# srinix007/GaussianProcessRegression.jl

Measured on AMD Instinct MI355X. Metric: GP-fit+predict wall-time and K-build GB/s + POTRF TFLOP/s at N=32768, higher is better.
Workload: dtype f64; 1 GPU; C3 fit+posterior: SE+SE+WN, N=32768, d=8, np=8192; N=32768, d=8, np=8192, kernel=SE+SE+WN, nb=128, parallelism=replicas x1

## Files before the change

gaussianprocessregression.jl_amd/csrc/dag.hip:

```cpp
#include <algorithm>
#include <cstdint>

#include "common.hpp"

#ifdef DAG_TRACE
__device__ unsigned long long g_diag_ph[16];
#define DSTAMP_INIT() unsigned long long _dst_t = __builtin_amdgcn_s_memrealtime()
#define DSTAMP(i)                                                   \
  do {                                                              \
    __syncthreads();                                                \
    if (threadIdx.x == 0) {                                         \
      const unsigned long long _t = __builtin_amdgcn_s_memrealtime(); \
      atomicAdd(&g_diag_ph[i], _t - _dst_t);                        \
      if ((i) == 7) atomicAdd(&g_diag_ph[8], 1ull);                 \
      _dst_t = _t;                                                  \
    }                                                               \
  } while (0)
#define DSTAMPW(i)                                                  \
  do {                                                              \
    const unsigned long long _t = __builtin_amdgcn_s_memrealtime(); \
    if (threadIdx.x == 0) atomicAdd(&g_diag_ph[i], _t - _dst_t);    \
    _dst_t = _t;                                                    \
  } while (0)
extern "C" void gpr_debug_diag_phases(unsigned long long* out, int reset) {
  hipMemcpyFromSymbol(out, HIP_SYMBOL(g_diag_ph), sizeof(unsigned long long) * 16);
  if (reset) {
    unsigned long long z[16] = {};
    hipMemcpyToSymbol(HIP_SYMBOL(g_diag_ph), z, sizeof z);
  }
}
#endif

#include "diag_block.hpp"

#ifdef DAG_TRACE
__device__ int g_dag_trace[4096];
#define DTRACE(slot, v)                                                                   \
  do {                                                                                    \
    if (__builtin_amdgcn_readfirstlane(threadIdx.x >> 6) == 0)                            \
      __hip_atomic_store(&g_dag_trace[blockIdx.x * 8 + (slot)], (v), __ATOMIC_RELAXED,     \
                         __HIP_MEMORY_SCOPE_SYSTEM);                                      \
  } while (0)
extern "C" void gpr_debug_dag_trace(int* out, void* stream) {
  hipMemcpyFromSymbolAsync(out, HIP_SYMBOL(g_dag_trace), sizeof(int) * 4096, 0,
                           hipMemcpyDeviceToHost, (hipStream_t)stream);
  hipStreamSynchronize((hipStream_t)stream);
}
#define PROF(var, ...)                                  \
  do {                                                  \
    const unsigned long long _t0 = __builtin_amdgcn_s_memrealtime(); \
    __VA_ARGS__;                                        \
    var += __builtin_amdgcn_s_memrealtime() - _t0;      \
  } while (0)
#else
#define DTRACE(slot, v) \
  do {                  \
  } while (0)
#define PROF(var, ...) \
  do {                 \
    __VA_ARGS__;       \
  } while (0)
#endif

namespace {

constexpr int DT = 128;
constexpr int DTK = 16;
#ifndef DAG_DPB
#define DAG_DPB 5
#endif
static_assert(DAG_DPB == 4 || DAG_DPB == 5, "dag_accum is written for 4 or 5 LDS stages");
constexpr int DPB = DAG_DPB;
constexpr int DSTAGE = (DT + DT) * DTK;
constexpr int DLDS = DPB * DSTAGE;
constexpr int DINT = (DLDS + 2) * 8 <= 160 * 1024 ? DLDS : DLDS - 2;
constexpr int DALLOC = DINT + 2;
constexpr int DNCH = DTK / 2;
constexpr int DRPD = 64 / DNCH;
constexpr int DNDMA = DT / (4 * DRPD);
constexpr int DVM = 2 * DNDMA;
constexpr int DNP = DTK / 8;
static_assert(D2_LDS_QTAIL <= DLDS, "diagonal block must fit in the stage buffers");

typedef double d2 __attribute__((ext_vector_type(2)));

struct DagArgs {
  double* A;
  size_t lda;
  int n, nt;
  double* B;
  size_t ldb;
  int nrhs, ntr;
  double* winv;
  int kglob;
  int* info;
  int* sync;
  int* ustored;
  const unsigned* tasks;
  int ntasks;
  int lower;
  double* G;
  size_t ldg;
  int gbase;
  long long spin_limit;
  int mirror;
  const int* tbatch;
  size_t strA, strB, strW;
  int strS;
};

__device__ __forceinline__ int ld_sc1(const int* p) {
  return __hip_atomic_load(p, __ATOMIC_RELAXED, __HIP_MEMORY_SCOPE_AGENT);
}

template <int VM>
__device__ __forceinline__ void dag_vmcnt() {
  asm volatile("s_waitcnt vmcnt(%0)" ::"n"(VM) : "memory");
}

__device__ __forceinline__ int dag_swz(int row) { return (row >> 1) & 7; }
__device__ __forceinline__ int dag_idx(int row, int chunk) {
  return row * DTK + ((chunk ^ dag_swz(row)) << 1);
}

__device__ __forceinline__ int dag_mblk(int wm, int j) {
  return 4 * (j >> 1) + (wm ? 1 + (j & 1) : 3 * (j & 1));
}

template <bool TRI = false>
__device__ __forceinline__ void dag_accum(d4v (&acc)[4][4], const double* __restrict__ P,
                                          size_t ldp, int mv, const double* __restrict__ Q,
                                          size_t ldq, int nv, int nst, double* lds) {
  if (nst <= 0) return;
  const int tid = threadIdx.x, lane = tid & 63;
  const int w = __builtin_amdgcn_readfirstlane(tid >> 6);
  const int wm = w & 1, wn = w >> 1;
  const double* srcP[DNDMA];
  const double* srcQ[DNDMA];
#pragma unroll
  for (int r = 0; r < DNDMA; ++r) {
    const int row = DRPD * (4 * r + w) + lane / DNCH;
    const int c = (lane % DNCH) ^ dag_swz(row);
    srcP[r] = P + 2 * c + (size_t)min(row, mv - 1) * ldp;
    srcQ[r] = Q + 2 * c + (size_t)min(row, nv - 1) * ldq;
  }
  auto issue = [&](int s, int b) {
    double* base = lds + b * DSTAGE;
    const size_t ko = (size_t)min(s, nst - 1) * DTK;
#pragma unroll
    for (int r = 0; r < DNDMA; ++r) {
      __builtin_amdgcn_global_load_lds(srcP[r] + ko, base + (4 * r + w) * 128, 16, 0, 0);
      __builtin_amdgcn_global_load_lds(srcQ[r] + ko, base + DT * DTK + (4 * r + w) * 128, 16, 0, 0);
    }
  };
  auto read_frags = [&](d2 (&F)[DNP][8], int b) {
    const double* ps = lds + b * DSTAGE;
    const double* qs = ps + DT * DTK;
#pragma unroll
    for (int p = 0; p < DNP; ++p) {
      const int ch = (lane >> 4) + 4 * p;
#pragma unroll
      for (int i = 0; i < 4; ++i)
        F[p][i] = *reinterpret_cast<const d2*>(&qs[dag_idx(wn * 64 + i * 16 + (lane & 15), ch)]);
#pragma unroll
      for (int j = 0; j < 4; ++j) {
        const int mrow = TRI ? 16 * dag_mblk(wm, j) : wm * 64 + j * 16;
        F[p][4 + j] = *reinterpret_cast<const d2*>(&ps[dag_idx(mrow + (lane & 15), ch)]);
      }
    }
  };
  auto mfma_stage = [&](const d2 (&F)[DNP][8], int s) {
    (void)s;
#pragma unroll
    for (int j = 0; j < 4; ++j) {
      if (TRI && dag_mblk(wm, j) < s) continue;
#pragma unroll
      for (int p = 0; p < DNP; ++p)
#pragma unroll
        for (int h = 0; h < 2; ++h)
#pragma unroll
          for (int i = 0; i < 4; ++i)
            acc[i][j] = __builtin_amdgcn_mfma_f64_16x16x4f64(F[p][i][h], F[p][4 + j][h], acc[i][j], 0, 0, 0);
    }
  };
#if DAG_DPB == 5
  d2 F0[DNP][8], F1[DNP][8];
  auto ring = [](int b, int k) { return b + k >= DPB ? b + k - DPB : b + k; };
  auto period = [&](int s, int b) {
    __builtin_amdgcn_sched_barrier(0);
    __builtin_amdgcn_s_waitcnt(0xC07F);
    dag_vmcnt<DVM>();
    __builtin_amdgcn_s_barrier();
    issue(s + 4, ring(b, 4));
    read_frags(F1, ring(b, 1));
    mfma_stage(F0, s);
    if constexpr (!TRI) {
      __builtin_amdgcn_sched_group_barrier(0x008, 1, 0);
#pragma unroll
      for (int t = 0; t < DVM; ++t) {
        __builtin_amdgcn_sched_group_barrier(0x020, 1, 0);
        __builtin_amdgcn_sched_group_barrier(0x008, 2, 0);
      }
#pragma unroll
      for (int t = 0; t < 8 * DNP; ++t) {
        __builtin_amdgcn_sched_group_barrier(0x100, 1, 0);
        __builtin_amdgcn_sched_group_barrier(0x008, 2, 0);
      }
      __builtin_amdgcn_sched_group_barrier(0x008, 32 * DNP - 1 - 2 * DVM - 16 * DNP, 0);
    }
    issue(s + 5, b);
    read_frags(F0, ring(b, 2));
    mfma_stage(F1, s + 1);
    if constexpr (!TRI) {
#pragma unroll
      for (int t = 0; t < DVM; ++t) {
        __builtin_amdgcn_sched_group_barrier(0x020, 1, 0);
        __builtin_amdgcn_sched_group_barrier(0x008, 2, 0);
      }
#pragma unroll
      for (int t = 0; t < 8 * DNP; ++t) {
        __builtin_amdgcn_sched_group_barrier(0x100, 1, 0);
        __builtin_amdgcn_sched_group_barrier(0x008, 2, 0);
      }
      __builtin_amdgcn_sched_group_barrier(0x008, 32 * DNP - 2 * DVM - 16 * DNP, 0);
    }
  };
#pragma unroll
  for (int t = 0; t < DPB - 1; ++t) issue(t, t);
  dag_vmcnt<DVM * (DPB - 2)>();
  __builtin_amdgcn_s_barrier();
  read_frags(F0, 0);
  __builtin_amdgcn_s_waitcnt(0xC07F);
  int s = 0;
  for (int b = 0; s + 1 < nst; s += 2, b = ring(b, 2)) period(s, b);
#else
  auto step = [&](int s, d2 (&Fc)[DNP][8], d2 (&Fn)[DNP][8]) {
    __builtin_amdgcn_sched_barrier(0);
    __builtin_amdgcn_s_waitcnt(0xC07F);
    dag_vmcnt<DVM * (DPB - 3)>();
    __builtin_amdgcn_s_barrier();
    issue(s + DPB - 1, (s + DPB - 1) % DPB);
    read_frags(Fn, (s + 1) % DPB);
    mfma_stage(Fc, s);
    if constexpr (TRI) return;
#ifndef DAG_SCHED
#define DAG_SCHED 0
#endif
#if DAG_SCHED == 0
#pragma unroll
    for (int t = 0; t < DVM; ++t) {
      __builtin_amdgcn_sched_group_barrier(0x020, 1, 0);
      __builtin_amdgcn_sched_group_barrier(0x008, 1, 0);
    }
#pragma unroll
    for (int t = 0; t < 8 * DNP; ++t) {
      __builtin_amdgcn_sched_group_barrier(0x100, 1, 0);
      __builtin_amdgcn_sched_group_barrier(0x008, 2, 0);
    }
    __builtin_amdgcn_sched_group_barrier(0x008, 32 * DNP - DVM - 16 * DNP, 0);
#elif DAG_SCHED == 1
#pragma unroll
    for (int t = 0; t < DVM; ++t) {
      __builtin_amdgcn_sched_group_barrier(0x020, 1, 0);
      __builtin_amdgcn_sched_group_barrier(0x008, 2, 0);
    }
#pragma unroll
    for (int t = 0; t < 8 * DNP; ++t) {
      __builtin_amdgcn_sched_group_barrier(0x100, 1, 0);
      __builtin_amdgcn_sched_group_barrier(0x008, 2, 0);
    }
    __builtin_amdgcn_sched_group_barrier(0x008, 32 * DNP - 2 * DVM - 16 * DNP, 0);
#elif DAG_SCHED == 2
#pragma unroll
    for (int t = 0; t < 8 * DNP; ++t) {
      __builtin_amdgcn_sched_group_barrier(0x100, 1, 0);
      __builtin_amdgcn_sched_group_barrier(0x008, 1, 0);
    }
#pragma unroll
    for (int t = 0; t < DVM; ++t) {
      __builtin_amdgcn_sched_group_barrier(0x020, 1, 0);
      __builtin_amdgcn_sched_group_barrier(0x008, 2, 0);
    }
    __builtin_amdgcn_sched_group_barrier(0x008, 32 * DNP - 2 * DVM - 8 * DNP, 0);
#endif
  };
  d2 F0[DNP][8], F1[DNP][8];
#pragma unroll
  for (int t = 0; t < DPB - 1; ++t) issue(t, t);
  dag_vmcnt<DVM * (DPB - 2)>();
  __builtin_amdgcn_s_barrier();
  read_frags(F0, 0);
  __builtin_amdgcn_s_waitcnt(0xC07F);
  int s = 0;
  for (; s + 1 < nst; s += 2) {
    step(s, F0, F1);
    step(s + 1, F1, F0);
  }
#endif
  if (s < nst) mfma_stage(F0, s);
  dag_vmcnt<0>();
  __syncthreads();
}


__device__ __forceinline__ int dag_wait(const int* pa, const int* pb, int have, int cap,
                                        int* info, long long limit, int* sh) {
  if (__builtin_amdgcn_readfirstlane(threadIdx.x >> 6) == 0) {
    int v = 0;
    long long spins = 0;
    for (;;) {
      v = __builtin_amdgcn_readfirstlane(min(ld_sc1(pa), ld_sc1(pb)));
      if (v > have) break;
      if (++spins > limit) {
        atomicCAS(info, 0, -1);
        v = cap;
        break;
      }
      __builtin_amdgcn_s_sleep(2);
    }
    *sh = min(v, cap);
  }
  __builtin_amdgcn_fence(__ATOMIC_ACQUIRE, "workgroup");
  __syncthreads();
  const int r = __builtin_amdgcn_readfirstlane(*sh);
  __syncthreads();
  return r;
}

__device__ __forceinline__ void dag_publish(int* prog, int v) {
  asm volatile("s_waitcnt vmcnt(0)" ::: "memory");
  __syncthreads();
  if (__builtin_amdgcn_readfirstlane(threadIdx.x >> 6) == 0)
    __hip_atomic_store(prog, v, __ATOMIC_RELAXED, __HIP_MEMORY_SCOPE_AGENT);
}
// ... 47 lines not shown
#pragma unroll
  for (int ii = 0; ii < 4; ++ii)
#pragma unroll
    for (int r = 0; r < 4; ++r) {
      const int nn = wn * 64 + ii * 16 + (lane >> 4) + 4 * r;
#pragma unroll
      for (int jj = 0; jj < 4; ++jj) {
        const int mm = wm * 64 + jj * 16 + (lane & 15);
        if (mm < mv && nn < nv && (i != j || mm <= nn))
          T[(size_t)mm + (size_t)nn * a.ldg] = acc[ii][jj][r];
      }
    }
  double* Tm = a.G + (size_t)j * DT + (size_t)i * DT * a.ldg;
#pragma unroll
  for (int ii = 0; ii < 4; ++ii)
#pragma unroll
    for (int jj = 0; jj < 4; ++jj)
#pragma unroll
      for (int r = 0; r < 4; ++r) {
        const int nn = wn * 64 + ii * 16 + (lane >> 4) + 4 * r;
        const int mm = wm * 64 + jj * 16 + (lane & 15);
        if (mm < mv && nn < nv && (i != j || mm < nn))
          Tm[(size_t)nn + (size_t)mm * a.ldg] = acc[ii][jj][r];
      }
}

template <bool GRAM, bool BATCH>
__global__ __launch_bounds__(256, 1) void potrf_dag_kernel(DagArgs a0) {
  DagArgs a = a0;
  __shared__ double lds[DALLOC];
  int& s_task = reinterpret_cast<int*>(lds + DINT)[0];
  int& s_skip = reinterpret_cast<int*>(lds + DINT)[1];
  int& s_wait = reinterpret_cast<int*>(lds + DINT)[2];
  int s_fok = 0;
  const int tid = threadIdx.x, lane = tid & 63;
  const int w = __builtin_amdgcn_readfirstlane(tid >> 6);
  const int wm = w & 1, wn = w >> 1;
  int* colprog = a.sync + 2;
  int* rhsprog = colprog + a.nt;
  unsigned long long p_wait = 0, p_acc = 0, p_fac = 0, p_tri = 0, p_all = 0, p_n = 0;
#ifdef DAG_PROF_PUB
  unsigned long long p_pub = 0, p_tri_unused = 0;
#define p_tri p_tri_unused
#endif
  (void)p_wait; (void)p_acc; (void)p_fac; (void)p_tri; (void)p_all; (void)p_n;
#ifdef DAG_TRACE
  const unsigned long long p_start = __builtin_amdgcn_s_memrealtime();
#endif
  for (;;) {
    if (w == 0) {
      const int tk = atomicAdd(&a0.sync[0], lane == 0 ? 1 : 0);
      const int tk0 = __builtin_amdgcn_readlane(tk, 0);
      s_task = tk0;
      if (!BATCH) {
        s_skip = __builtin_amdgcn_readfirstlane(ld_sc1(a.info)) != 0;
      } else if (tk0 < a0.ntasks) {
        const int b = __builtin_amdgcn_readfirstlane(a0.tbatch[tk0]);
        s_skip = __builtin_amdgcn_readfirstlane(ld_sc1(a0.info + b)) != 0;
      }
    }
    __syncthreads();
    const int t = __builtin_amdgcn_readfirstlane(s_task);
    const bool skip = __builtin_amdgcn_readfirstlane(s_skip);
    DTRACE(0, t);
    DTRACE(1, 1);
    if (t >= a.ntasks) break;
    if (BATCH) {
      const int b = __builtin_amdgcn_readfirstlane(a0.tbatch[t]);
      a.A = a0.A + (size_t)b * a0.strA;
      a.B = a0.B + (size_t)b * a0.strB;
      a.winv = a0.winv + (size_t)b * a0.strW;
      a.info = a0.info + b;
      colprog = a0.sync + (size_t)b * a0.strS + 2;
      rhsprog = colprog + a.nt;
    }
    const unsigned code = __builtin_amdgcn_readfirstlane(a.tasks[t]);
    if (GRAM && t >= a.gbase) {
      if (!skip) dag_gram_task(a, (code >> 16) & 0x7fff, code & 0xffff, lds, &s_wait, p_wait, p_acc);
      ++p_n;
      __syncthreads();
      continue;
    }
    const bool rhs = code >> 31;
    const int i = (code >> 16) & 0x7fff, j = code & 0xffff;
    const bool diag = !rhs && i == j;
    double* T = rhs ? a.B + (size_t)i * DT + (size_t)j * DT * a.ldb
                    : a.A + (size_t)i * DT + (size_t)j * DT * a.lda;
    const size_t ldt = rhs ? a.ldb : a.lda;
    const double* Qcol = rhs ? a.B + (size_t)j * DT * a.ldb : a.A + (size_t)j * DT * a.lda;
    const double* Pcol = a.A + (size_t)i * DT * a.lda;
    int* pj = rhs ? rhsprog + j : colprog + j;
    const int mv = min(DT, a.n - i * DT);
    const int nv = min(DT, (rhs ? a.nrhs : a.n) - j * DT);
    if (!skip) {
      d4v acc[4][4];
#pragma unroll
      for (int ii = 0; ii < 4; ++ii)
#pragma unroll
        for (int r = 0; r < 4; ++r) {
          const int nn = wn * 64 + ii * 16 + (lane >> 4) + 4 * r;
          const double* col = T + (size_t)min(nn, nv - 1) * ldt;
#pragma unroll
          for (int jj = 0; jj < 4; ++jj) {
            const int mm = wm * 64 + jj * 16 + (lane & 15);
            const double c = col[min(mm, mv - 1)];
            acc[ii][jj][r] = (mm < mv && nn < nv) ? -c : 0.0;
          }
        }
      if (a.mirror && !rhs && !diag) {
        double* Tm = a.A + (size_t)j * DT + (size_t)i * DT * a.lda;
#pragma unroll
        for (int ii = 0; ii < 4; ++ii)
#pragma unroll
          for (int jj = 0; jj < 4; ++jj)
#pragma unroll
            for (int r = 0; r < 4; ++r) {
              const int nn = wn * 64 + ii * 16 + (lane >> 4) + 4 * r;
              const int mm = wm * 64 + jj * 16 + (lane & 15);
              if (mm < mv && nn < nv) Tm[(size_t)nn + (size_t)mm * a.lda] = -acc[ii][jj][r];
            }
      }
      DTRACE(1, 2);
      int done = (rhs && a.lower) ? j : 0;
      while (done < i) {
        int r = 0;
        PROF(p_wait, r = dag_wait(colprog + i, pj, done, i, a.info, a.spin_limit, &s_wait));
        PROF(p_acc, dag_accum(acc, Pcol + (size_t)done * DT, a.lda, mv, Qcol + (size_t)done * DT,
                              ldt, nv, (r - done) * (DT / DTK), lds));
        done = r;
      }
      if (diag) {
        double* S = lds;
#pragma unroll
        for (int ii = 0; ii < 4; ++ii)
#pragma unroll
          for (int r = 0; r < 4; ++r) {
            const int nn = wn * 64 + ii * 16 + (lane >> 4) + 4 * r;
#pragma unroll
            for (int jj = 0; jj < 4; ++jj) {
              const int mm = wm * 64 + jj * 16 + (lane & 15);
              if (mm <= nn) S[pk(mm, nn)] = nn < mv ? -acc[ii][jj][r] : (mm == nn ? 1.0 : 0.0);
            }
          }
        __syncthreads();
        DTRACE(1, 3);
        int f = 0;
        PROF(p_fac, f = dag_factor(S, mv, a.kglob + i * DT, a.winv + (size_t)i * DT * DT));
        if (f && w == 0) atomicCAS(a.info, 0, f);
        s_fok = f == 0;
        DTRACE(1, 4);
      } else {
        if (i > 0) {
#pragma unroll
          for (int ii = 0; ii < 4; ++ii)
#pragma unroll
            for (int r = 0; r < 4; ++r) {
              const int nn = wn * 64 + ii * 16 + (lane >> 4) + 4 * r;
#pragma unroll
              for (int jj = 0; jj < 4; ++jj) {
                const int mm = wm * 64 + jj * 16 + (lane & 15);
                if (mm < mv && nn < nv) T[(size_t)mm + (size_t)nn * ldt] = -acc[ii][jj][r];
              }
            }
        }
        asm volatile("s_waitcnt vmcnt(0)" ::: "memory");
        __builtin_amdgcn_fence(__ATOMIC_RELEASE, "workgroup");
        PROF(p_wait, dag_wait(colprog + i, colprog + i, i, i + 1, a.info, a.spin_limit, &s_wait));
#pragma unroll
        for (int ii = 0; ii < 4; ++ii)
#pragma unroll
          for (int jj = 0; jj < 4; ++jj) acc[ii][jj] = d4v{0.0, 0.0, 0.0, 0.0};
        const bool tri = mv == DT;
        if (tri)
          PROF(p_tri, dag_accum<true>(acc, a.winv + (size_t)i * DT * DT, DT, mv, T, ldt, nv, DT / DTK, lds));
        else
          PROF(p_tri, dag_accum(acc, a.winv + (size_t)i * DT * DT, DT, mv, T, ldt, nv, mv / DTK, lds));
#pragma unroll
        for (int ii = 0; ii < 4; ++ii)
#pragma unroll
          for (int r = 0; r < 4; ++r) {
            const int nn = wn * 64 + ii * 16 + (lane >> 4) + 4 * r;
#pragma unroll
            for (int jj = 0; jj < 4; ++jj) {
              const int mm = (tri ? 16 * dag_mblk(wm, jj) : wm * 64 + jj * 16) + (lane & 15);
              if (mm < mv && nn < nv) st_res<true>(&T[(size_t)mm + (size_t)nn * ldt], acc[ii][jj][r]);
            }
          }
      }
    } else if (a.mirror && !rhs && !diag) {
      double* Tm = a.A + (size_t)j * DT + (size_t)i * DT * a.lda;
      for (int e = tid; e < DT * DT; e += 256) {
        const int mm = e & (DT - 1), nn = e >> 7;
        if (mm < mv && nn < nv) Tm[(size_t)nn + (size_t)mm * a.lda] = T[(size_t)mm + (size_t)nn * ldt];
      }
    }
    DTRACE(1, 5);
#ifdef DAG_PROF_PUB
    if (diag) PROF(p_pub, dag_publish(pj, i + 1)); else dag_publish(pj, i + 1);
#else
    dag_publish(pj, i + 1);
#endif
    DTRACE(1, 6);
    if (diag && !skip && __builtin_amdgcn_readfirstlane(s_fok))
      dag_store_u(lds, T, a.lda, mv, a.ustored != nullptr);
    if (diag && a.ustored) dag_publish(a.ustored + i, 1);
    ++p_n;
  }
  DTRACE(1, 7);
#ifdef DAG_TRACE
  p_all = __builtin_amdgcn_s_memrealtime() - p_start;
  DTRACE(2, (int)p_wait);
  DTRACE(3, (int)p_acc);
  DTRACE(4, (int)p_fac);
#ifdef DAG_PROF_PUB
#undef p_tri
  DTRACE(5, (int)p_pub);
  (void)p_tri_unused;
#else
  DTRACE(5, (int)p_tri);
#endif
  DTRACE(6, (int)p_all);
  DTRACE(7, (int)p_n);
#endif
}

}

__global__ void dag_init_kernel(int* sync, int nt, int ntr, int solve, int lower) {
  for (int t = blockIdx.x * blockDim.x + threadIdx.x; t < nt + ntr; t += gridDim.x * blockDim.x)
    sync[2 + t] = t < nt ? (solve ? t + 1 : 0) : (lower ? t - nt : 0);
}

static long long dag_spin_limit(const gpr_ctx* ctx) {
#ifdef GPR_TESTING
  if (const char* sl = getenv("GPR_DAG_SPIN_LIMIT")) return std::max(1ll, atoll(sl));
#endif
  return ctx->dag_spin_limit;
}

bool dag_shape_ok(int n, int lda, const double* dA) {
  return n > 0 && n % 16 == 0 && lda % 16 == 0 && ((uintptr_t)dA & 127) == 0 && n <= DT * 32767;
}

bool dag_takes_whole(const gpr_ctx* ctx, int n, int lda, const double* dA) {
  (void)lda;
  (void)dA;
  return ctx->dag_mode && ctx->nb == DT && n > 0 &&
         n <= DT * 32767 - 16;
}

__global__ void dag_pad_in_kernel(const double* __restrict__ A, size_t lda, int n,
                                  double* __restrict__ W, int n2) {
  const size_t tot = (size_t)n2 * n2;
  for (size_t t = blockIdx.x * (size_t)blockDim.x + threadIdx.x; t < tot;
       t += (size_t)gridDim.x * blockDim.x) {
    const int r = (int)(t % n2), c = (int)(t / n2);
    if (r <= c) W[t] = c < n ? A[(size_t)r + (size_t)c * lda] : (r == c ? 1.0 : 0.0);
  }
}

__global__ void dag_pad_out_kernel(double* __restrict__ A, size_t lda, int n,
                                   const double* __restrict__ W, int n2) {
  const size_t tot = (size_t)n * n;
  for (size_t t = blockIdx.x * (size_t)blockDim.x + threadIdx.x; t < tot;
       t += (size_t)gridDim.x * blockDim.x) {
    const int r = (int)(t % n), c = (int)(t / n);
    if (r <= c) A[(size_t)r + (size_t)c * lda] = W[(size_t)r + (size_t)c * n2];
  }
}

int launch_potrf_dag_padded(gpr_ctx* ctx, double* dA, int n, int lda, double* dB, int nrhs,
                            int ldb) {
  const int n2 = (n + 15) / 16 * 16;
  hipStream_t st = ctx->stream;
// ... 3 lines not shown
    (void)hipGetLastError();
    return 1;
  }
  const int blocks = 2048;
  dag_pad_in_kernel<<<blocks, 256, 0, st>>>(dA, (size_t)lda, n, ctx->dpadA, n2);
  LAUNCH_CHECK(ctx);
  if (dB) {
    HIP_TRY(ctx, hipMemcpy2DAsync(ctx->dpadB, (size_t)n2 * sizeof(double), dB,
                                  (size_t)ldb * sizeof(double), (size_t)n * sizeof(double), nrhs,
                                  hipMemcpyDeviceToDevice, st));
    if (n2 > n)
      HIP_TRY(ctx, hipMemset2DAsync(ctx->dpadB + n, (size_t)n2 * sizeof(double), 0,
                                    (size_t)(n2 - n) * sizeof(double), nrhs, st));
  }
  const int rc = launch_potrf_dag(ctx, ctx->dpadA, n2, n2, dB ? ctx->dpadB : nullptr, nrhs, n2, 0,
                                  st, 0);
  if (rc) return rc < 0 ? rc : set_err(ctx, GPR_E_HIP, "padded tile-DAG: shape not eligible");
  dag_pad_out_kernel<<<blocks, 256, 0, st>>>(dA, (size_t)lda, n, ctx->dpadA, n2);
  LAUNCH_CHECK(ctx);
  if (dB)
    HIP_TRY(ctx, hipMemcpy2DAsync(dB, (size_t)ldb * sizeof(double), ctx->dpadB,
                                  (size_t)n2 * sizeof(double), (size_t)n * sizeof(double), nrhs,
                                  hipMemcpyDeviceToDevice, st));
  return 0;
}

int launch_potrf_dag(gpr_ctx* ctx, double* dA, int n, int lda, double* dB, int nrhs, int ldb,
                     int kglob, hipStream_t st, int flags, double* dG, int ldg) {
  const bool solve = flags & DAG_SOLVE, lower = flags & DAG_LOWER, gram = flags & DAG_GRAM;
  const bool mirror = flags & DAG_MIRROR;
  if ((solve || lower) && (!dB || kglob)) return 1;
  if (mirror && (solve || kglob)) return 1;
  if (gram && (!lower || !dG || ldg < n || nrhs != n)) return 1;
  if (ctx->nb != DT || n <= 0 || n % 16 || lda % 16 || ((uintptr_t)dA & 127) || n > DT * 32767 ||
      kglob % DT)
    return 1;
  if (dB && (nrhs <= 0 || ldb % 16 || ((uintptr_t)dB & 127) || nrhs > DT * 65535)) return 1;
  const int nt = (n + DT - 1) / DT, ntr = dB ? (nrhs + DT - 1) / DT : 0;
  GPR_TRY(ensure_winv(ctx, kglob + n, DT));
  if (ctx->dag_nt != nt || ctx->dag_ntr != ntr || ctx->dag_flags != (flags & ~DAG_MIRROR) ||
      ctx->dag_lag_built != ctx->dag_zlag) {
    std::vector<unsigned> tasks;
    tasks.reserve((size_t)nt * (nt + 1) + (size_t)nt * ntr);
    const int lag = solve || !lower ? 0 : std::min(ctx->dag_zlag, nt);
    auto rhs_row = [&](int i) {
      for (int c = 0; c < (lower ? std::min(ntr, i + 1) : ntr); ++c)
        tasks.push_back(0x80000000u | ((unsigned)i << 16) | (unsigned)c);
    };
    for (int i = 0; i < nt; ++i) {
      if (!solve)
        for (int j = i; j < nt; ++j) tasks.push_back(((unsigned)i << 16) | (unsigned)j);
      if (i - lag >= 0) rhs_row(i - lag);
    }
    for (int i = std::max(nt - lag, 0); i < nt; ++i) rhs_row(i);
    if (gram)
      for (int j = 0; j < nt; ++j)
        for (int i = 0; i <= j; ++i) tasks.push_back(((unsigned)i << 16) | (unsigned)j);
    if (ctx->dag_tasks) {
      HIP_TRY(ctx, hipStreamSynchronize(ctx->stream));
      HIP_TRY(ctx, hipFree(ctx->dag_tasks));
    }
    ctx->dag_tasks = nullptr;
    ctx->dag_nt = ctx->dag_ntr = -1;
    HIP_TRY(ctx, hipMalloc((void**)&ctx->dag_tasks, tasks.size() * sizeof(unsigned)));
    HIP_TRY(ctx, hipMemcpy(ctx->dag_tasks, tasks.data(), tasks.size() * sizeof(unsigned),
                           hipMemcpyHostToDevice));
    ctx->dag_ntasks = (int)tasks.size();
    ctx->dag_nt = nt;
    ctx->dag_ntr = ntr;
    ctx->dag_flags = flags & ~DAG_MIRROR;
// ... 58 lines not shown
      hook_ev = nullptr;
    }
    (void)hipGetLastError();
  }
  const double flops = (solve ? 0.0 : (double)n * n * n / 3.0) +
                       (lower ? (double)n * n * n / 3.0 : (double)n * n * (dB ? nrhs : 0)) +
                       (gram ? (double)n * n * n / 3.0 : 0.0);
  {
    hipStream_t ls = ctx->ls;
    ctx->ls = st;
    TimerScope ts(ctx, solve ? TC_DAG_SOLVE : TC_DAG, flops);
    if (gram)
      potrf_dag_kernel<true, false><<<grid, 256, 0, st>>>(a);
    else
      potrf_dag_kernel<false, false><<<grid, 256, 0, st>>>(a);
    ctx->ls = ls;
    const hipError_t le = hipGetLastError();
    if (le != hipSuccess) {
      if (hook_ev) hipEventDestroy(hook_ev);
      return set_err(ctx, GPR_E_HIP, "tile-DAG launch: %s", hipGetErrorString(le));
    }
  }
  if (hook) {
    hook(ctx->dag_hook_user, dA, n, lda, ctx->dag_sync + 2, a.ustored, nt, hook_ev);
    if (hook_ev) hipEventDestroy(hook_ev);
  }
  return 0;
}

int launch_potrf_dag_batch(gpr_ctx* ctx, double* dA, size_t strA, int n, int lda, double* dB,
                           size_t strB, int nrhs, int ldb, int nbatch, int* info_out) {
  hipStream_t st = ctx->stream;
  if (nbatch <= 0) return 0;
  if (n <= 0 || n % 16 || lda % 16 || strA % 16 || ((uintptr_t)dA & 127) || n > DT * 32767)
    return 1;
  if (dB && (nrhs <= 0 || ldb % 16 || strB % 16 || ((uintptr_t)dB & 127) || nrhs > DT * 65535))
    return 1;
  const int nt = (n + DT - 1) / DT, ntr = dB ? (nrhs + DT - 1) / DT : 0;
  std::vector<unsigned> tasks;
  std::vector<int> tb;
  const size_t per = (size_t)nt * (nt + 1) / 2 + (size_t)nt * ntr;
  tasks.reserve(per * nbatch);
  tb.reserve(per * nbatch);
  for (int i = 0; i < nt; ++i) {
    for (int b = 0; b < nbatch; ++b)
      for (int j = i; j < nt; ++j) {
        tasks.push_back(((unsigned)i << 16) | (unsigned)j);
        tb.push_back(b);
      }
    for (int b = 0; b < nbatch; ++b)
      for (int c = 0; c < ntr; ++c) {
        tasks.push_back(0x80000000u | ((unsigned)i << 16) | (unsigned)c);
        tb.push_back(b);
      }
  }
  const int ntasks = (int)tasks.size();
  const int strS = 2 + nt + ntr;
  const size_t nW = (size_t)nbatch * nt * DT * DT;
  const size_t nI = (size_t)ntasks * 2 + (size_t)nbatch * strS + (size_t)nbatch;
  GPR_TRY(ensure_buf(ctx, &ctx->dagb, &ctx->dagb_cap, nW + (nI + 1) / 2 + 1));
  double* W = ctx->dagb;
  unsigned* dtasks = reinterpret_cast<unsigned*>(W + nW);
  int* dtb = reinterpret_cast<int*>(dtasks + ntasks);
  int* dsync = dtb + ntasks;
  int* dinfo = dsync + (size_t)nbatch * strS;
  HIP_TRY(ctx, hipMemcpyAsync(dtasks, tasks.data(), sizeof(unsigned) * ntasks, hipMemcpyHostToDevice, st));
  HIP_TRY(ctx, hipMemcpyAsync(dtb, tb.data(), sizeof(int) * ntasks, hipMemcpyHostToDevice, st));
  HIP_TRY(ctx, hipMemsetAsync(dsync, 0, sizeof(int) * ((size_t)nbatch * strS + nbatch), st));
  if (ctx->ncu <= 0) {
// ... 44 lines not shown
```

Baseline: 3.349 GP jobs/s (fit N=32768 + posterior mean/var np=8192, per GPU).

## Stage triangular-solve Q operand directly into LDS instead of via global round-trip

For full-size diagonal-triangle tiles in the DAG Cholesky/TRSM kernel, the negated accumulator is written straight into the LDS Q stages of the ring buffer rather than stored to global memory and reloaded. The prologue then only DMAs the W-inverse (P) operand, and the first period waits on fewer outstanding loads. The task-code and batch-index loads are also hoisted into the ticket-fetch wave to save a reload. Extra trace instrumentation is added under DAG_TRACE. This relies on LDS stage layout matching the swizzle and on T no longer being written to global for that wave half, which is a correctness risk.

```diff
diff --git a/gaussianprocessregression.jl_amd/csrc/dag.hip b/gaussianprocessregression.jl_amd/csrc/dag.hip
--- a/gaussianprocessregression.jl_amd/csrc/dag.hip
+++ b/gaussianprocessregression.jl_amd/csrc/dag.hip
@@ -1,5 +1,6 @@
 #include <algorithm>
 #include <cstdint>
+#include <type_traits>
 
 #include "common.hpp"
 
@@ -52,13 +53,44 @@
     __VA_ARGS__;                                        \
     var += __builtin_amdgcn_s_memrealtime() - _t0;      \
   } while (0)
+__device__ int g_dag_trace2[4096];
+#define DTRACE2(slot, v)                                                                  \
+  do {                                                                                    \
+    if (__builtin_amdgcn_readfirstlane(threadIdx.x >> 6) == 0)                            \
+      __hip_atomic_store(&g_dag_trace2[blockIdx.x * 8 + (slot)], (v), __ATOMIC_RELAXED,    \
+                         __HIP_MEMORY_SCOPE_SYSTEM);                                      \
+  } while (0)
+extern "C" void gpr_debug_dag_trace2(int* out, void* stream) {
+  hipMemcpyFromSymbolAsync(out, HIP_SYMBOL(g_dag_trace2), sizeof(int) * 4096, 0,
+                           hipMemcpyDeviceToHost, (hipStream_t)stream);
+  hipStreamSynchronize((hipStream_t)stream);
+}
+#define PLAP0() (_lap = __builtin_amdgcn_s_memrealtime())
+#define PLAP(var)                                                   \
+  do {                                                              \
+    const unsigned long long _t = __builtin_amdgcn_s_memrealtime(); \
+    var += _t - _lap;                                               \
+    _lap = _t;                                                      \
+  } while (0)
+#define PDRAIN() asm volatile("s_waitcnt vmcnt(0)" ::: "memory")
+#define P_WPRO &p_wpro
 #else
+#define P_WPRO nullptr
 #define DTRACE(slot, v) \
   do {                  \
   } while (0)
 #define PROF(var, ...) \
   do {                 \
     __VA_ARGS__;       \
+  } while (0)
+#define PLAP0() \
+  do {          \
+  } while (0)
+#define PLAP(var) \
+  do {            \
+  } while (0)
+#define PDRAIN() \
+  do {           \
   } while (0)
 #endif
 
@@ -127,11 +159,16 @@
   return 4 * (j >> 1) + (wm ? 1 + (j & 1) : 3 * (j & 1));
 }
 
-template <bool TRI = false>
+template <bool TRI = false, bool QL = false>
 __device__ __forceinline__ void dag_accum(d4v (&acc)[4][4], const double* __restrict__ P,
                                           size_t ldp, int mv, const double* __restrict__ Q,
-                                          size_t ldq, int nv, int nst, double* lds) {
+                                          size_t ldq, int nv, int nst, double* lds,
+                                          unsigned long long* p_pro = nullptr) {
   if (nst <= 0) return;
+#ifdef DAG_TRACE
+  const unsigned long long t_in = __builtin_amdgcn_s_memrealtime();
+#endif
+  (void)p_pro;
   const int tid = threadIdx.x, lane = tid & 63;
   const int w = __builtin_amdgcn_readfirstlane(tid >> 6);
   const int wm = w & 1, wn = w >> 1;
@@ -153,6 +190,12 @@
       __builtin_amdgcn_global_load_lds(srcQ[r] + ko, base + DT * DTK + (4 * r + w) * 128, 16, 0, 0);
     }
   };
+  auto issue_p = [&](int s, int b) {
+    double* base = lds + b * DSTAGE;
+#pragma unroll
+    for (int r = 0; r < DNDMA; ++r)
+      __builtin_amdgcn_global_load_lds(srcP[r] + (size_t)s * DTK, base + (4 * r + w) * 128, 16, 0, 0);
+  };
   auto read_frags = [&](d2 (&F)[DNP][8], int b) {
     const double* ps = lds + b * DSTAGE;
     const double* qs = ps + DT * DTK;
@@ -186,10 +229,10 @@
 #if DAG_DPB == 5
   d2 F0[DNP][8], F1[DNP][8];
   auto ring = [](int b, int k) { return b + k >= DPB ? b + k - DPB : b + k; };
-  auto period = [&](int s, int b) {
+  auto period = [&](int s, int b, auto first) {
     __builtin_amdgcn_sched_barrier(0);
     __builtin_amdgcn_s_waitcnt(0xC07F);
-    dag_vmcnt<DVM>();
+    dag_vmcnt<(QL && decltype(first)::value) ? DNDMA : DVM>();
     __builtin_amdgcn_s_barrier();
     issue(s + 4, ring(b, 4));
     read_frags(F1, ring(b, 1));
@@ -225,14 +268,28 @@
       __builtin_amdgcn_sched_group_barrier(0x008, 32 * DNP - 2 * DVM - 16 * DNP, 0);
     }
   };
-#pragma unroll
-  for (int t = 0; t < DPB - 1; ++t) issue(t, t);
-  dag_vmcnt<DVM * (DPB - 2)>();
+  static_assert(!QL || TRI, "LDS-resident Q stages: the W-product only (nst = 8 > DPB - 1)");
+#pragma unroll
+  for (int t = 0; t < DPB - 1; ++t) {
+    if constexpr (QL)
+      issue_p(t, t);
+    else
+      issue(t, t);
+  }
+  dag_vmcnt<(QL ? DNDMA : DVM) * (DPB - 2)>();
   __builtin_amdgcn_s_barrier();
   read_frags(F0, 0);
   __builtin_amdgcn_s_waitcnt(0xC07F);
-  int s = 0;
-  for (int b = 0; s + 1 < nst; s += 2, b = ring(b, 2)) period(s, b);
+#ifdef DAG_TRACE
+  if (p_pro) *p_pro += __builtin_amdgcn_s_memrealtime() - t_in;
+#endif
+  int s = 0, b = 0;
+  if constexpr (QL) {
+    period(0, 0, std::true_type{});
+    s = 2;
+    b = 2;
+  }
+  for (; s + 1 < nst; s += 2, b = ring(b, 2)) period(s, b, std::false_type{});
 #else
   auto step = [&](int s, d2 (&Fc)[DNP][8], d2 (&Fn)[DNP][8]) {
     __builtin_amdgcn_sched_barrier(0);
@@ -284,6 +341,7 @@
     __builtin_amdgcn_sched_group_barrier(0x008, 32 * DNP - 2 * DVM - 8 * DNP, 0);
 #endif
   };
+  static_assert(!QL, "LDS-resident Q stages: the ring of five only");
   d2 F0[DNP][8], F1[DNP][8];
 #pragma unroll
   for (int t = 0; t < DPB - 1; ++t) issue(t, t);
@@ -300,6 +358,24 @@
   if (s < nst) mfma_stage(F0, s);
   dag_vmcnt<0>();
   __syncthreads();
+}
+
+#ifndef DAG_Q_LDS
+#define DAG_Q_LDS 1
+#endif
+constexpr bool DAG_QLDS = DAG_DPB == 5 && DAG_Q_LDS;
+__device__ __forceinline__ void dag_q_to_lds(const d4v (&acc)[4][4], double* lds, int wn, int lane) {
+  int l = lane;
+  asm volatile("" : "+v"(l));
+  const int kk = l & 15;
+#pragma unroll
+  for (int r = 0; r < 4; ++r) {
+    double* q = lds + DT * DTK + dag_idx(wn * 64 + (l >> 4) + 4 * r, kk >> 1) + (kk & 1);
+#pragma unroll
+    for (int ii = 0; ii < 4; ++ii)
+#pragma unroll
+      for (int jj = 0; jj < 4; ++jj) q[jj * DSTAGE + ii * 16 * DTK] = -acc[ii][jj][r];
+  }
 }
 
 
@@ -413,6 +489,7 @@
   int& s_task = reinterpret_cast<int*>(lds + DINT)[0];
   int& s_skip = reinterpret_cast<int*>(lds + DINT)[1];
   int& s_wait = reinterpret_cast<int*>(lds + DINT)[2];
+  int& s_code = reinterpret_cast<int*>(lds + DINT)[3];
   int s_fok = 0;
   const int tid = threadIdx.x, lane = tid & 63;
   const int w = __builtin_amdgcn_readfirstlane(tid >> 6);
@@ -427,27 +504,32 @@
   (void)p_wait; (void)p_acc; (void)p_fac; (void)p_tri; (void)p_all; (void)p_n;
 #ifdef DAG_TRACE
   const unsigned long long p_start = __builtin_amdgcn_s_memrealtime();
+  unsigned long long p_tkt = 0, p_ld = 0, p_mir = 0, p_bst = 0, p_wpro = 0, p_fin = 0, _lap = 0;
 #endif
   for (;;) {
+    PLAP0();
     if (w == 0) {
       const int tk = atomicAdd(&a0.sync[0], lane == 0 ? 1 : 0);
       const int tk0 = __builtin_amdgcn_readlane(tk, 0);
       s_task = tk0;
-      if (!BATCH) {
-        s_skip = __builtin_amdgcn_readfirstlane(ld_sc1(a.info)) != 0;
-      } else if (tk0 < a0.ntasks) {
-        const int b = __builtin_amdgcn_readfirstlane(a0.tbatch[tk0]);
-        s_skip = __builtin_amdgcn_readfirstlane(ld_sc1(a0.info + b)) != 0;
+      if (tk0 < a0.ntasks) {
+        const int b = BATCH ? __builtin_amdgcn_readfirstlane(a0.tbatch[tk0]) : 0;
+        const unsigned cd = a0.tasks[tk0];
+        const int sk = ld_sc1(a0.info + b);
+        s_code = __builtin_amdgcn_readfirstlane(cd);
+        s_skip = (__builtin_amdgcn_readfirstlane(sk) != 0) | (b << 1);
       }
     }
     __syncthreads();
     const int t = __builtin_amdgcn_readfirstlane(s_task);
-    const bool skip = __builtin_amdgcn_readfirstlane(s_skip);
+    const int skipb = __builtin_amdgcn_readfirstlane(s_skip);
+    const bool skip = skipb & 1;
+    const unsigned code = __builtin_amdgcn_readfirstlane(s_code);
     DTRACE(0, t);
     DTRACE(1, 1);
     if (t >= a.ntasks) break;
     if (BATCH) {
-      const int b = __builtin_amdgcn_readfirstlane(a0.tbatch[t]);
+      const int b = skipb >> 1;
       a.A = a0.A + (size_t)b * a0.strA;
       a.B = a0.B + (size_t)b * a0.strB;
       a.winv = a0.winv + (size_t)b * a0.strW;
@@ -455,7 +537,7 @@
       colprog = a0.sync + (size_t)b * a0.strS + 2;
       rhsprog = colprog + a.nt;
     }
-    const unsigned code = __builtin_amdgcn_readfirstlane(a.tasks[t]);
+    PLAP(p_tkt);
     if (GRAM && t >= a.gbase) {
       if (!skip) dag_gram_task(a, (code >> 16) & 0x7fff, code & 0xffff, lds, &s_wait, p_wait, p_acc);
       ++p_n;
@@ -488,6 +570,8 @@
             acc[ii][jj][r] = (mm < mv && nn < nv) ? -c : 0.0;
           }
         }
+      PDRAIN();
+      PLAP(p_ld);
       if (a.mirror && !rhs && !diag) {
         double* Tm = a.A + (size_t)j * DT + (size_t)i * DT * a.lda;
 #pragma unroll
@@ -500,6 +584,8 @@
               const int mm = wm * 64 + jj * 16 + (lane & 15);
               if (mm < mv && nn < nv) Tm[(size_t)nn + (size_t)mm * a.lda] = -acc[ii][jj][r];
             }
+        PDRAIN();
+        PLAP(p_mir);
       }
       DTRACE(1, 2);
       int done = (rhs && a.lower) ? j : 0;
@@ -530,8 +616,13 @@
         if (f && w == 0) atomicCAS(a.info, 0, f);
         s_fok = f == 0;
         DTRACE(1, 4);
+        PLAP0();
       } else {
-        if (i > 0) {
+        PLAP0();
+        const bool tri = mv == DT;
+        const bool qlds = DAG_QLDS && tri;
+        if (qlds && wm == 0) dag_q_to_lds(acc, lds, wn, lane);
+        if (i > 0 && !(qlds && wm == 0)) {
 #pragma unroll
           for (int ii = 0; ii < 4; ++ii)
 #pragma unroll
@@ -544,18 +635,21 @@
               }
             }
         }
-        asm volatile("s_waitcnt vmcnt(0)" ::: "memory");
+        if (!qlds) asm volatile("s_waitcnt vmcnt(0)" ::: "memory");
         __builtin_amdgcn_fence(__ATOMIC_RELEASE, "workgroup");
+        PLAP(p_bst);
         PROF(p_wait, dag_wait(colprog + i, colprog + i, i, i + 1, a.info, a.spin_limit, &s_wait));
 #pragma unroll
         for (int ii = 0; ii < 4; ++ii)
 #pragma unroll
           for (int jj = 0; jj < 4; ++jj) acc[ii][jj] = d4v{0.0, 0.0, 0.0, 0.0};
-        const bool tri = mv == DT;
         if (tri)
-          PROF(p_tri, dag_accum<true>(acc, a.winv + (size_t)i * DT * DT, DT, mv, T, ldt, nv, DT / DTK, lds));
+          PROF(p_tri, dag_accum<true, DAG_QLDS>(acc, a.winv + (size_t)i * DT * DT, DT, mv, T, ldt, nv,
+                                                DT / DTK, lds, P_WPRO));
         else
-          PROF(p_tri, dag_accum(acc, a.winv + (size_t)i * DT * DT, DT, mv, T, ldt, nv, mv / DTK, lds));
+          PROF(p_tri, dag_accum(acc, a.winv + (size_t)i * DT * DT, DT, mv, T, ldt, nv, mv / DTK, lds,
+                                P_WPRO));
+        PLAP0();
 #pragma unroll
         for (int ii = 0; ii < 4; ++ii)
 #pragma unroll
@@ -576,12 +670,16 @@
       }
     }
     DTRACE(1, 5);
+#ifdef DAG_TRACE
+    if (skip) PLAP0();
+#endif
 #ifdef DAG_PROF_PUB
     if (diag) PROF(p_pub, dag_publish(pj, i + 1)); else dag_publish(pj, i + 1);
 #else
     dag_publish(pj, i + 1);
 #endif
     DTRACE(1, 6);
+    PLAP(p_fin);
     if (diag && !skip && __builtin_amdgcn_readfirstlane(s_fok))
       dag_store_u(lds, T, a.lda, mv, a.ustored != nullptr);
     if (diag && a.ustored) dag_publish(a.ustored + i, 1);
@@ -602,6 +700,12 @@
 #endif
   DTRACE(6, (int)p_all);
   DTRACE(7, (int)p_n);
+  DTRACE2(0, (int)p_tkt);
+  DTRACE2(1, (int)p_ld);
+  DTRACE2(2, (int)p_mir);
+  DTRACE2(3, (int)p_bst);
+  DTRACE2(4, (int)p_wpro);
+  DTRACE2(5, (int)p_fin);
 #endif
 }
 
```

Measured after the change: 3.362 GP jobs/s (fit N=32768 + posterior mean/var np=8192, per GPU), median of 6. About the same (+0.4%).

## Hand-schedule DAG GEMM inner loop with inline-asm LDS DMA and precomputed addresses

Applied to the files above, without the earlier changes.

Rewrites the dag_accum inner pipeline. Global-to-LDS loads now go through inline asm with a scalar base and a 32-bit per-lane offset, and LDS fragment addresses are precomputed. The 5-stage ring is fully unrolled with compile-time buffer indices, and DMA pieces are interleaved explicitly between MFMAs. The aim is to cut per-iteration address arithmetic and VGPR pressure and to get a tighter MFMA/DMA interleave. In exchange it adds a leading-dimension limit so the 32-bit offsets stay valid (larger lda falls back off the DAG path), drops the 4-stage variant, and carries the risks of hand-written m0 asm.

```diff
diff --git a/gaussianprocessregression.jl_amd/csrc/dag.hip b/gaussianprocessregression.jl_amd/csrc/dag.hip
--- a/gaussianprocessregression.jl_amd/csrc/dag.hip
+++ b/gaussianprocessregression.jl_amd/csrc/dag.hip
@@ -1,5 +1,6 @@
 #include <algorithm>
 #include <cstdint>
+#include <type_traits>
 
 #include "common.hpp"
 
@@ -66,11 +67,8 @@
 
 constexpr int DT = 128;
 constexpr int DTK = 16;
-#ifndef DAG_DPB
-#define DAG_DPB 5
-#endif
-static_assert(DAG_DPB == 4 || DAG_DPB == 5, "dag_accum is written for 4 or 5 LDS stages");
-constexpr int DPB = DAG_DPB;
+constexpr int DPB = 5;
+constexpr int DAG_LD_MAX = 1 << 25;
 constexpr int DSTAGE = (DT + DT) * DTK;
 constexpr int DLDS = DPB * DSTAGE;
 constexpr int DINT = (DLDS + 2) * 8 <= 160 * 1024 ? DLDS : DLDS - 2;
@@ -127,176 +125,167 @@
   return 4 * (j >> 1) + (wm ? 1 + (j & 1) : 3 * (j & 1));
 }
 
+typedef __attribute__((address_space(3))) const char* dag_ldsp;
+
+__device__ __forceinline__ void dag_dma16(unsigned voff, const char* sbase, unsigned lds_dst) {
+  unsigned keep;
+  asm volatile(
+      "s_mov_b32 %0, m0\n\ts_mov_b32 m0, %3\n\ts_nop 0\n\tglobal_load_lds_dwordx4 %1, %2\n\ts_mov_b32 m0, %0"
+      : "=&s"(keep)
+      : "v"(voff), "s"(sbase), "s"(lds_dst)
+      : "memory");
+}
+
+__device__ __forceinline__ const char* dag_uniform(const void* p) {
+  const unsigned long long v = (unsigned long long)(uintptr_t)p;
+  const unsigned lo = __builtin_amdgcn_readfirstlane((unsigned)v);
+  const unsigned hi = __builtin_amdgcn_readfirstlane((unsigned)(v >> 32));
+  return reinterpret_cast<const char*>((uintptr_t)(((unsigned long long)hi << 32) | lo));
+}
+
 template <bool TRI = false>
 __device__ __forceinline__ void dag_accum(d4v (&acc)[4][4], const double* __restrict__ P,
                                           size_t ldp, int mv, const double* __restrict__ Q,
                                           size_t ldq, int nv, int nst, double* lds) {
   if (nst <= 0) return;
+  static_assert(DPB == 5 && DNDMA == 4 && DNP == 2, "the unrolled ring is written for this shape");
+  using std::integral_constant;
   const int tid = threadIdx.x, lane = tid & 63;
   const int w = __builtin_amdgcn_readfirstlane(tid >> 6);
   const int wm = w & 1, wn = w >> 1;
-  const double* srcP[DNDMA];
-  const double* srcQ[DNDMA];
+  const char* gP[DNDMA];
+  const char* gQ[DNDMA];
+  unsigned oP[DNDMA], oQ[DNDMA];
 #pragma unroll
   for (int r = 0; r < DNDMA; ++r) {
-    const int row = DRPD * (4 * r + w) + lane / DNCH;
-    const int c = (lane % DNCH) ^ dag_swz(row);
-    srcP[r] = P + 2 * c + (size_t)min(row, mv - 1) * ldp;
-    srcQ[r] = Q + 2 * c + (size_t)min(row, nv - 1) * ldq;
-  }
-  auto issue = [&](int s, int b) {
-    double* base = lds + b * DSTAGE;
-    const size_t ko = (size_t)min(s, nst - 1) * DTK;
-#pragma unroll
-    for (int r = 0; r < DNDMA; ++r) {
-      __builtin_amdgcn_global_load_lds(srcP[r] + ko, base + (4 * r + w) * 128, 16, 0, 0);
-      __builtin_amdgcn_global_load_lds(srcQ[r] + ko, base + DT * DTK + (4 * r + w) * 128, 16, 0, 0);
-    }
+    const int row0 = DRPD * (4 * r + w), row = row0 + lane / DNCH;
+    const unsigned c16 = 16u * ((lane % DNCH) ^ dag_swz(row));
+    const int p0 = min(row0, mv - 1), q0 = min(row0, nv - 1);
+    gP[r] = dag_uniform(P + (size_t)p0 * ldp);
+    gQ[r] = dag_uniform(Q + (size_t)q0 * ldq);
+    oP[r] = c16 + (unsigned)(min(row, mv - 1) - p0) * (unsigned)(8 * ldp);
+    oQ[r] = c16 + (unsigned)(min(row, nv - 1) - q0) * (unsigned)(8 * ldq);
+    asm volatile("" : "+v"(oP[r]), "+v"(oQ[r]));
+  }
+  const unsigned lds0 = __builtin_amdgcn_readfirstlane((unsigned)(uintptr_t)(dag_ldsp)lds);
+  auto piece = [&](int t, int s, int bb) __attribute__((always_inline)) {
+    const size_t ko = (size_t)min(s, nst - 1) * (DTK * 8);
+    const int r = t >> 1;
+    const unsigned dst = lds0 + bb * (DSTAGE * 8) + (t & 1) * (DT * DTK * 8) + (4 * r + w) * 1024;
+    if (t & 1)
+      dag_dma16(oQ[r], gQ[r] + ko, dst);
+    else
+      dag_dma16(oP[r], gP[r] + ko, dst);
   };
-  auto read_frags = [&](d2 (&F)[DNP][8], int b) {
-    const double* ps = lds + b * DSTAGE;
-    const double* qs = ps + DT * DTK;
-#pragma unroll
-    for (int p = 0; p < DNP; ++p) {
-      const int ch = (lane >> 4) + 4 * p;
-#pragma unroll
-      for (int i = 0; i < 4; ++i)
-        F[p][i] = *reinterpret_cast<const d2*>(&qs[dag_idx(wn * 64 + i * 16 + (lane & 15), ch)]);
-#pragma unroll
-      for (int j = 0; j < 4; ++j) {
-        const int mrow = TRI ? 16 * dag_mblk(wm, j) : wm * 64 + j * 16;
-        F[p][4 + j] = *reinterpret_cast<const d2*>(&ps[dag_idx(mrow + (lane & 15), ch)]);
-      }
-    }
+  constexpr int NJP = TRI ? 2 : 1;
+  dag_ldsp qb[DNP][3], pb[DNP][NJP][3];
+  {
+    const int l15 = lane & 15;
+    const unsigned a0 = 8u * (unsigned)dag_idx(l15, lane >> 4);
+#pragma unroll
+    for (int p = 0; p < DNP; ++p)
+#pragma unroll
+      for (int k = 0; k < 3; ++k) {
+        const unsigned ap = (a0 ^ (64u * p)) + 65536u * k;
+        qb[p][k] = (dag_ldsp)lds + DT * DTK * 8 + wn * (64 * DTK * 8) + ap;
+        asm volatile("" : "+v"(qb[p][k]));
+#pragma unroll
+        for (int jp = 0; jp < NJP; ++jp) {
+          pb[p][jp][k] = (dag_ldsp)lds + (TRI ? 16 * DTK * 8 * (wm ? 1 + jp : 3 * jp) : wm * (64 * DTK * 8)) + ap;
+          asm volatile("" : "+v"(pb[p][jp][k]));
+        }
+      }
+  }
+  typedef __attribute__((address_space(3))) const d2* ldsd2;
+  auto rd = [&](d2 (&F)[DNP][8], int t, int bb) __attribute__((always_inline)) {
+    const int p = t >> 3, f = t & 7, j = f & 3;
+    const int win = (bb & 1) * (DSTAGE * 8);
+    if (f < 4)
+      F[p][f] = *reinterpret_cast<ldsd2>(qb[p][bb >> 1] + win + j * (16 * DTK * 8));
+    else if (TRI)
+      F[p][f] = *reinterpret_cast<ldsd2>(pb[p][j & (NJP - 1)][bb >> 1] + win + (j >> 1) * (64 * DTK * 8));
+    else
+      F[p][f] = *reinterpret_cast<ldsd2>(pb[p][0][bb >> 1] + win + j * (16 * DTK * 8));
   };
-  auto mfma_stage = [&](const d2 (&F)[DNP][8], int s) {
+  auto mf = [&](const d2 (&F)[DNP][8], int t) __attribute__((always_inline)) {
+    const int j = t >> 4, p = (t >> 3) & 1, h = (t >> 2) & 1, i = t & 3;
+    acc[i][j] = __builtin_amdgcn_mfma_f64_16x16x4f64(F[p][i][h], F[p][4 + j][h], acc[i][j], 0, 0, 0);
+  };
+  auto mfma_stage = [&](const d2 (&F)[DNP][8], int s) __attribute__((always_inline)) {
     (void)s;
 #pragma unroll
     for (int j = 0; j < 4; ++j) {
       if (TRI && dag_mblk(wm, j) < s) continue;
 #pragma unroll
-      for (int p = 0; p < DNP; ++p)
-#pragma unroll
-        for (int h = 0; h < 2; ++h)
-#pragma unroll
-          for (int i = 0; i < 4; ++i)
-            acc[i][j] = __builtin_amdgcn_mfma_f64_16x16x4f64(F[p][i][h], F[p][4 + j][h], acc[i][j], 0, 0, 0);
+      for (int t = 16 * j; t < 16 * j + 16; ++t) mf(F, t);
     }
   };
-#if DAG_DPB == 5
+  auto half = [&](const d2 (&Fc)[DNP][8], d2 (&Fn)[DNP][8], int s, int sd, int bd, int br,
+                  auto leadc) __attribute__((always_inline)) {
+    constexpr int LEAD = decltype(leadc)::value;
+    if constexpr (TRI) {
+#pragma unroll
+      for (int t = 0; t < DVM; ++t) piece(t, sd, bd);
+#pragma unroll
+      for (int t = 0; t < 8 * DNP; ++t) rd(Fn, t, br);
+      mfma_stage(Fc, s);
+    } else {
+      int m = 0;
+#pragma unroll
+      for (; m < LEAD; ++m) mf(Fc, m);
+#pragma unroll
+      for (int t = 0; t < DVM; ++t) {
+        __builtin_amdgcn_sched_barrier(0);
+        piece(t, sd, bd);
+        mf(Fc, m++);
+        mf(Fc, m++);
+      }
+      __builtin_amdgcn_sched_barrier(0);
+#pragma unroll
+      for (int t = 0; t < 8 * DNP; ++t) rd(Fn, t, br);
+#pragma unroll
+      for (; m < 32 * DNP; ++m) mf(Fc, m);
+#pragma unroll
+      for (int t = 0; t < 8 * DNP; ++t) {
+        __builtin_amdgcn_sched_group_barrier(0x100, 1, 0);
+        __builtin_amdgcn_sched_group_barrier(0x008, 2, 0);
+      }
+      __builtin_amdgcn_sched_group_barrier(0x008, 32 * DNP - LEAD - 2 * DVM - 16 * DNP, 0);
+    }
+  };
   d2 F0[DNP][8], F1[DNP][8];
-  auto ring = [](int b, int k) { return b + k >= DPB ? b + k - DPB : b + k; };
-  auto period = [&](int s, int b) {
+  int s = 0;
+  auto period = [&](auto bc) __attribute__((always_inline)) {
+    constexpr int B = decltype(bc)::value;
     __builtin_amdgcn_sched_barrier(0);
     __builtin_amdgcn_s_waitcnt(0xC07F);
     dag_vmcnt<DVM>();
     __builtin_amdgcn_s_barrier();
-    issue(s + 4, ring(b, 4));
-    read_frags(F1, ring(b, 1));
-    mfma_stage(F0, s);
-    if constexpr (!TRI) {
-      __builtin_amdgcn_sched_group_barrier(0x008, 1, 0);
-#pragma unroll
-      for (int t = 0; t < DVM; ++t) {
-        __builtin_amdgcn_sched_group_barrier(0x020, 1, 0);
-        __builtin_amdgcn_sched_group_barrier(0x008, 2, 0);
-      }
-#pragma unroll
-      for (int t = 0; t < 8 * DNP; ++t) {
-        __builtin_amdgcn_sched_group_barrier(0x100, 1, 0);
-        __builtin_amdgcn_sched_group_barrier(0x008, 2, 0);
-      }
-      __builtin_amdgcn_sched_group_barrier(0x008, 32 * DNP - 1 - 2 * DVM - 16 * DNP, 0);
-    }
-    issue(s + 5, b);
-    read_frags(F0, ring(b, 2));
-    mfma_stage(F1, s + 1);
-    if constexpr (!TRI) {
-#pragma unroll
-      for (int t = 0; t < DVM; ++t) {
-        __builtin_amdgcn_sched_group_barrier(0x020, 1, 0);
-        __builtin_amdgcn_sched_group_barrier(0x008, 2, 0);
-      }
-#pragma unroll
-      for (int t = 0; t < 8 * DNP; ++t) {
-        __builtin_amdgcn_sched_group_barrier(0x100, 1, 0);
-        __builtin_amdgcn_sched_group_barrier(0x008, 2, 0);
-      }
-      __builtin_amdgcn_sched_group_barrier(0x008, 32 * DNP - 2 * DVM - 16 * DNP, 0);
-    }
+    half(F0, F1, s, s + 4, (B + 4) % DPB, (B + 1) % DPB, integral_constant<int, 1>{});
+    half(F1, F0, s + 1, s + 5, B, (B + 2) % DPB, integral_constant<int, 0>{});
+    s += 2;
   };
 #pragma unroll
-  for (int t = 0; t < DPB - 1; ++t) issue(t, t);
+  for (int t = 0; t < DPB - 1; ++t)
+#pragma unroll
+    for (int u = 0; u < DVM; ++u) piece(u, t, t);
   dag_vmcnt<DVM * (DPB - 2)>();
   __builtin_amdgcn_s_barrier();
-  read_frags(F0, 0);
+#pragma unroll
+  for (int t = 0; t < 8 * DNP; ++t) rd(F0, t, 0);
   __builtin_amdgcn_s_waitcnt(0xC07F);
-  int s = 0;
-  for (int b = 0; s + 1 < nst; s += 2, b = ring(b, 2)) period(s, b);
-#else
-  auto step = [&](int s, d2 (&Fc)[DNP][8], d2 (&Fn)[DNP][8]) {
-    __builtin_amdgcn_sched_barrier(0);
-    __builtin_amdgcn_s_waitcnt(0xC07F);
-    dag_vmcnt<DVM * (DPB - 3)>();
-    __builtin_amdgcn_s_barrier();
-    issue(s + DPB - 1, (s + DPB - 1) % DPB);
-    read_frags(Fn, (s + 1) % DPB);
-    mfma_stage(Fc, s);
-    if constexpr (TRI) return;
-#ifndef DAG_SCHED
-#define DAG_SCHED 0
-#endif
-#if DAG_SCHED == 0
-#pragma unroll
-    for (int t = 0; t < DVM; ++t) {
-      __builtin_amdgcn_sched_group_barrier(0x020, 1, 0);
-      __builtin_amdgcn_sched_group_barrier(0x008, 1, 0);
-    }
-#pragma unroll
-    for (int t = 0; t < 8 * DNP; ++t) {
-      __builtin_amdgcn_sched_group_barrier(0x100, 1, 0);
-      __builtin_amdgcn_sched_group_barrier(0x008, 2, 0);
-    }
-    __builtin_amdgcn_sched_group_barrier(0x008, 32 * DNP - DVM - 16 * DNP, 0);
-#elif DAG_SCHED == 1
-#pragma unroll
-    for (int t = 0; t < DVM; ++t) {
-      __builtin_amdgcn_sched_group_barrier(0x020, 1, 0);
-      __builtin_amdgcn_sched_group_barrier(0x008, 2, 0);
-    }
-#pragma unroll
-    for (int t = 0; t < 8 * DNP; ++t) {
-      __builtin_amdgcn_sched_group_barrier(0x100, 1, 0);
-      __builtin_amdgcn_sched_group_barrier(0x008, 2, 0);
-    }
-    __builtin_amdgcn_sched_group_barrier(0x008, 32 * DNP - 2 * DVM - 16 * DNP, 0);
-#elif DAG_SCHED == 2
-#pragma unroll
-    for (int t = 0; t < 8 * DNP; ++t) {
-      __builtin_amdgcn_sched_group_barrier(0x100, 1, 0);
-      __builtin_amdgcn_sched_group_barrier(0x008, 1, 0);
-    }
-#pragma unroll
-    for (int t = 0; t < DVM; ++t) {
-      __builtin_amdgcn_sched_group_barrier(0x020, 1, 0);
-      __builtin_amdgcn_sched_group_barrier(0x008, 2, 0);
-    }
-    __builtin_amdgcn_sched_group_barrier(0x008, 32 * DNP - 2 * DVM - 8 * DNP, 0);
-#endif
-  };
-  d2 F0[DNP][8], F1[DNP][8];
-#pragma unroll
-  for (int t = 0; t < DPB - 1; ++t) issue(t, t);
-  dag_vmcnt<DVM * (DPB - 2)>();
-  __builtin_amdgcn_s_barrier();
-  read_frags(F0, 0);
-  __builtin_amdgcn_s_waitcnt(0xC07F);
-  int s = 0;
-  for (; s + 1 < nst; s += 2) {
-    step(s, F0, F1);
-    step(s + 1, F1, F0);
-  }
-#endif
+  int np = nst >> 1;
+  for (; np >= 5; np -= 5) {
+    period(integral_constant<int, 0>{});
+    period(integral_constant<int, 2>{});
+    period(integral_constant<int, 4>{});
+    period(integral_constant<int, 1>{});
+    period(integral_constant<int, 3>{});
+  }
+  if (np > 0) period(integral_constant<int, 0>{});
+  if (np > 1) period(integral_constant<int, 2>{});
+  if (np > 2) period(integral_constant<int, 4>{});
+  if (np > 3) period(integral_constant<int, 1>{});
   if (s < nst) mfma_stage(F0, s);
   dag_vmcnt<0>();
   __syncthreads();
@@ -620,7 +609,12 @@
 }
 
 bool dag_shape_ok(int n, int lda, const double* dA) {
-  return n > 0 && n % 16 == 0 && lda % 16 == 0 && ((uintptr_t)dA & 127) == 0 && n <= DT * 32767;
+  return n > 0 && n % 16 == 0 && lda % 16 == 0 && lda <= DAG_LD_MAX && ((uintptr_t)dA & 127) == 0 &&
+         n <= DT * 32767;
+}
+
+extern "C" int gpr_debug_dag_shape_ok(int n, int lda, unsigned long long addr) {
+  return dag_shape_ok(n, lda, reinterpret_cast<const double*>((uintptr_t)addr)) ? 1 : 0;
 }
 
 bool dag_takes_whole(const gpr_ctx* ctx, int n, int lda, const double* dA) {
@@ -690,10 +684,11 @@
   if ((solve || lower) && (!dB || kglob)) return 1;
   if (mirror && (solve || kglob)) return 1;
   if (gram && (!lower || !dG || ldg < n || nrhs != n)) return 1;
-  if (ctx->nb != DT || n <= 0 || n % 16 || lda % 16 || ((uintptr_t)dA & 127) || n > DT * 32767 ||
-      kglob % DT)
+  if (ctx->nb != DT || n <= 0 || n % 16 || lda % 16 || lda > DAG_LD_MAX || ((uintptr_t)dA & 127) ||
+      n > DT * 32767 || kglob % DT)
     return 1;
-  if (dB && (nrhs <= 0 || ldb % 16 || ((uintptr_t)dB & 127) || nrhs > DT * 65535)) return 1;
+  if (dB && (nrhs <= 0 || ldb % 16 || ldb > DAG_LD_MAX || ((uintptr_t)dB & 127) || nrhs > DT * 65535))
+    return 1;
   const int nt = (n + DT - 1) / DT, ntr = dB ? (nrhs + DT - 1) / DT : 0;
   GPR_TRY(ensure_winv(ctx, kglob + n, DT));
   if (ctx->dag_nt != nt || ctx->dag_ntr != ntr || ctx->dag_flags != (flags & ~DAG_MIRROR) ||
@@ -818,9 +813,11 @@
                            size_t strB, int nrhs, int ldb, int nbatch, int* info_out) {
   hipStream_t st = ctx->stream;
   if (nbatch <= 0) return 0;
-  if (n <= 0 || n % 16 || lda % 16 || strA % 16 || ((uintptr_t)dA & 127) || n > DT * 32767)
+  if (n <= 0 || n % 16 || lda % 16 || lda > DAG_LD_MAX || strA % 16 || ((uintptr_t)dA & 127) ||
+      n > DT * 32767)
     return 1;
-  if (dB && (nrhs <= 0 || ldb % 16 || strB % 16 || ((uintptr_t)dB & 127) || nrhs > DT * 65535))
+  if (dB && (nrhs <= 0 || ldb % 16 || ldb > DAG_LD_MAX || strB % 16 || ((uintptr_t)dB & 127) ||
+             nrhs > DT * 65535))
     return 1;
   const int nt = (n + DT - 1) / DT, ntr = dB ? (nrhs + DT - 1) / DT : 0;
   std::vector<unsigned> tasks;
```

After: 3.307 GP jobs/s (fit N=32768 + posterior mean/var np=8192, per GPU) before, 3.358 GP jobs/s (fit N=32768 + posterior mean/var np=8192, per GPU) after, median of 6. 1.6% higher.
